# mkshing/e4t-diffusion

Measured on NVIDIA H100. Metric: E4T pretrain images/sec @512^2 bs16 SD-v1.4, higher is better.
Workload: dtype bf16

## Files before the change

e4t-diffusion_b200/csrc/common.cuh:

```cuda
#pragma once
#include <cuda.h>
#include <cuda_runtime.h>
#include <cuda_bf16.h>
#include <stdint.h>
#include <stdio.h>
#include <string.h>

typedef __nv_bfloat16 bf16;

extern thread_local char g_e4t_err[512];
int e4t_set_error(const char* fmt, ...);

#define E4T_CHECK(cond, ...)                                   \
  do {                                                         \
    if (!(cond)) return e4t_set_error(__VA_ARGS__);            \
  } while (0)

#define E4T_CUDA(call)                                                                  \
  do {                                                                                  \
    cudaError_t _e = (call);                                                            \
    if (_e != cudaSuccess)                                                              \
      return e4t_set_error("%s:%d CUDA error %s: %s", __FILE__, __LINE__, #call,        \
                           cudaGetErrorString(_e));                                     \
  } while (0)

#define E4T_LAUNCH_CHECK() E4T_CUDA(cudaGetLastError())

extern unsigned long long g_e4t_launches;
#define E4T_COUNT_LAUNCH() (++g_e4t_launches)

int e4t_tmap_encode(CUtensorMap* map, const void* gptr, int rank, const uint64_t* dims,
                    const uint64_t* strides_bytes ,
                    const uint32_t* box, int elem_bytes , int swizzle_bytes = 128,
                    const uint32_t* elem_strides = nullptr );

static inline int cdiv(long a, long b) { return (int)((a + b - 1) / b); }

#ifdef __CUDACC__
__device__ __forceinline__ uint32_t smem_u32(const void* p) {
  return static_cast<uint32_t>(__cvta_generic_to_shared(p));
}
__device__ __forceinline__ uint32_t lane_id() { return threadIdx.x & 31; }

__device__ __forceinline__ void mbar_init(uint64_t* bar, uint32_t count) {
  asm volatile("mbarrier.init.shared::cta.b64 [%0], %1;" ::"r"(smem_u32(bar)), "r"(count) : "memory");
}
__device__ __forceinline__ void fence_mbar_init() {
  asm volatile("fence.mbarrier_init.release.cluster;" ::: "memory");
}
__device__ __forceinline__ void mbar_expect_tx(uint64_t* bar, uint32_t bytes) {
  asm volatile("mbarrier.arrive.expect_tx.shared::cta.b64 _, [%0], %1;" ::"r"(smem_u32(bar)), "r"(bytes)
               : "memory");
}
__device__ __forceinline__ void mbar_arrive(uint64_t* bar) {
  asm volatile("mbarrier.arrive.shared::cta.b64 _, [%0];" ::"r"(smem_u32(bar)) : "memory");
}
__device__ __forceinline__ bool mbar_try_wait(uint64_t* bar, uint32_t parity) {
  uint32_t ok;
  asm volatile(
      "{\n\t.reg .pred p;\n\t"
      "mbarrier.try_wait.parity.shared::cta.b64 p, [%1], %2;\n\t"
      "selp.u32 %0, 1, 0, p;\n\t}"
      : "=r"(ok)
      : "r"(smem_u32(bar)), "r"(parity)
      : "memory");
  return ok != 0;
}
__device__ __forceinline__ bool mbar_test_wait(uint64_t* bar, uint32_t parity) {
  uint32_t ok;
  asm volatile(
      "{\n\t.reg .pred p;\n\t"
      "mbarrier.test_wait.parity.shared::cta.b64 p, [%1], %2;\n\t"
      "selp.u32 %0, 1, 0, p;\n\t}"
      : "=r"(ok)
      : "r"(smem_u32(bar)), "r"(parity)
      : "memory");
  return ok != 0;
}
__device__ __forceinline__ void mbar_wait(uint64_t* bar, uint32_t parity) {
  while (!mbar_try_wait(bar, parity)) {
  }
}

__device__ __forceinline__ void fence_proxy_async_smem() {
  asm volatile("fence.proxy.async.shared::cta;" ::: "memory");
}

__device__ __forceinline__ void tma_prefetch_desc(const CUtensorMap* m) {
  asm volatile("prefetch.tensormap [%0];" ::"l"(reinterpret_cast<uint64_t>(m)) : "memory");
}
__device__ __forceinline__ void tma_load_2d(void* smem, const CUtensorMap* m, uint64_t* bar, int c0, int c1) {
  asm volatile(
      "cp.async.bulk.tensor.2d.shared::cluster.global.mbarrier::complete_tx::bytes [%0], [%1, {%3, %4}], [%2];"
      ::"r"(smem_u32(smem)), "l"(reinterpret_cast<uint64_t>(m)), "r"(smem_u32(bar)), "r"(c0), "r"(c1)
      : "memory");
}
__device__ __forceinline__ void tma_load_3d(void* smem, const CUtensorMap* m, uint64_t* bar, int c0, int c1,
                                            int c2) {
  asm volatile(
      "cp.async.bulk.tensor.3d.shared::cluster.global.mbarrier::complete_tx::bytes [%0], [%1, {%3, %4, %5}], [%2];"
      ::"r"(smem_u32(smem)), "l"(reinterpret_cast<uint64_t>(m)), "r"(smem_u32(bar)), "r"(c0), "r"(c1), "r"(c2)
      : "memory");
}
__device__ __forceinline__ void tma_load_4d(void* smem, const CUtensorMap* m, uint64_t* bar, int c0, int c1,
                                            int c2, int c3) {
  asm volatile(
      "cp.async.bulk.tensor.4d.shared::cluster.global.mbarrier::complete_tx::bytes [%0], [%1, {%3, %4, %5, %6}], "
      "[%2];" ::"r"(smem_u32(smem)),
      "l"(reinterpret_cast<uint64_t>(m)), "r"(smem_u32(bar)), "r"(c0), "r"(c1), "r"(c2), "r"(c3)
      : "memory");
}

__device__ __forceinline__ void bulk_load_1d(void* smem, const void* g, uint32_t bytes, uint64_t* bar) {
  asm volatile("cp.async.bulk.shared::cluster.global.mbarrier::complete_tx::bytes [%0], [%1], %2, [%3];" ::"r"(
                   smem_u32(smem)),
               "l"(g), "r"(bytes), "r"(smem_u32(bar))
               : "memory");
}

__device__ __forceinline__ void tma_store_3d(const CUtensorMap* m, const void* smem, int c0, int c1, int c2) {
  asm volatile("cp.async.bulk.tensor.3d.global.shared::cta.bulk_group [%0, {%2, %3, %4}], [%1];" ::"l"(
                   reinterpret_cast<uint64_t>(m)),
               "r"(smem_u32(smem)), "r"(c0), "r"(c1), "r"(c2)
               : "memory");
}
__device__ __forceinline__ void tma_reduce_add_3d(const CUtensorMap* m, const void* smem, int c0, int c1, int c2) {
  asm volatile("cp.reduce.async.bulk.tensor.3d.global.shared::cta.add.tile.bulk_group [%0, {%2, %3, %4}], [%1];" ::"l"(
                   reinterpret_cast<uint64_t>(m)),
               "r"(smem_u32(smem)), "r"(c0), "r"(c1), "r"(c2)
               : "memory");
}
__device__ __forceinline__ void tma_store_commit() { asm volatile("cp.async.bulk.commit_group;" ::: "memory"); }
template <int N>
__device__ __forceinline__ void tma_store_wait_read() {
  asm volatile("cp.async.bulk.wait_group.read %0;" ::"n"(N) : "memory");
}
__device__ __forceinline__ void tma_store_wait_all() { asm volatile("cp.async.bulk.wait_group 0;" ::: "memory"); }

__device__ __forceinline__ uint64_t wgmma_desc(uint32_t saddr, uint32_t lbo_bytes, uint32_t sbo_bytes) {
  uint64_t d = 0;
  d |= (uint64_t)((saddr & 0x3FFFFu) >> 4);
  d |= (uint64_t)((lbo_bytes >> 4) & 0x3FFFu) << 16;
  d |= (uint64_t)((sbo_bytes >> 4) & 0x3FFFu) << 32;
  d |= 1ull << 62;
  return d;
}
__device__ __forceinline__ void wgmma_fence() { asm volatile("wgmma.fence.sync.aligned;" ::: "memory"); }
__device__ __forceinline__ void wgmma_commit() { asm volatile("wgmma.commit_group.sync.aligned;" ::: "memory"); }
template <int N>
__device__ __forceinline__ void wgmma_wait() {
  asm volatile("wgmma.wait_group.sync.aligned %0;" ::"n"(N) : "memory");
}
template <int R>
__device__ __forceinline__ void reg_fence(float* d) {
#pragma unroll
  for (int i = 0; i < R; ++i) asm volatile("" : "+f"(d[i])::"memory");
}
template <int R>
__device__ __forceinline__ void reg_fence_u32(uint32_t* a) {
#pragma unroll
  for (int i = 0; i < R; ++i) asm volatile("" : "+r"(a[i])::"memory");
}
__device__ __forceinline__ void named_bar_sync(uint32_t id, uint32_t nthreads) {
  asm volatile("bar.sync %0, %1;" ::"r"(id), "r"(nthreads) : "memory");
}
template <int R>
__device__ __forceinline__ void setmaxnreg_dec() {
  asm volatile("setmaxnreg.dec.sync.aligned.u32 %0;" ::"n"(R));
}
template <int R>
__device__ __forceinline__ void setmaxnreg_inc() {
  asm volatile("setmaxnreg.inc.sync.aligned.u32 %0;" ::"n"(R));
}

__device__ __forceinline__ void ldsm_x4(uint32_t addr, uint32_t* r) {
  asm volatile("ldmatrix.sync.aligned.m8n8.x4.shared.b16 {%0, %1, %2, %3}, [%4];"
               : "=r"(r[0]), "=r"(r[1]), "=r"(r[2]), "=r"(r[3])
               : "r"(addr));
}
__device__ __forceinline__ void ldsm_x4_t(uint32_t addr, uint32_t* r) {
  asm volatile("ldmatrix.sync.aligned.m8n8.x4.trans.shared.b16 {%0, %1, %2, %3}, [%4];"
               : "=r"(r[0]), "=r"(r[1]), "=r"(r[2]), "=r"(r[3])
               : "r"(addr));
}
__device__ __forceinline__ void mma16816(float* d, const uint32_t* a, const uint32_t* b) {
  asm volatile(
      "mma.sync.aligned.m16n8k16.row.col.f32.bf16.bf16.f32 {%0, %1, %2, %3}, {%4, %5, %6, %7}, {%8, %9}, "
      "{%0, %1, %2, %3};"
      : "+f"(d[0]), "+f"(d[1]), "+f"(d[2]), "+f"(d[3])
      : "r"(a[0]), "r"(a[1]), "r"(a[2]), "r"(a[3]), "r"(b[0]), "r"(b[1]));
}
__device__ __forceinline__ void cp_async16(uint32_t dst, const void* src, uint32_t src_bytes) {
  asm volatile("cp.async.cg.shared.global [%0], [%1], 16, %2;" ::"r"(dst), "l"(src), "r"(src_bytes) : "memory");
}
__device__ __forceinline__ void cp_async_commit() { asm volatile("cp.async.commit_group;" ::: "memory"); }
template <int N>
__device__ __forceinline__ void cp_async_wait() {
  asm volatile("cp.async.wait_group %0;" ::"n"(N) : "memory");
}

__device__ __forceinline__ uint32_t sw128_off(uint32_t r, uint32_t c16) {
  return r * 128u + ((c16 ^ (r & 7u)) << 4);
}

__device__ __forceinline__ float warp_sum(float v) {
#pragma unroll
  for (int o = 16; o > 0; o >>= 1) v += __shfl_xor_sync(0xffffffffu, v, o);
  return v;
}
__device__ __forceinline__ float warp_max(float v) {
#pragma unroll
  for (int o = 16; o > 0; o >>= 1) v = fmaxf(v, __shfl_xor_sync(0xffffffffu, v, o));
  return v;
}
__device__ __forceinline__ uint32_t pack_bf16(float a, float b) {
  __nv_bfloat162 t = __floats2bfloat162_rn(a, b);
  return *reinterpret_cast<uint32_t*>(&t);
}
__device__ __forceinline__ float2 unpack_bf16(uint32_t u) {
  __nv_bfloat162 t = *reinterpret_cast<__nv_bfloat162*>(&u);
  return __bfloat1622float2(t);
}
__device__ __forceinline__ float ex2_approx(float x) {
  float y;
  asm("ex2.approx.ftz.f32 %0, %1;" : "=f"(y) : "f"(x));
  return y;
}
__device__ __forceinline__ float silu_f(float x) { return x / (1.f + __expf(-x)); }
#endif
```

e4t-diffusion_b200/csrc/gemm.cu:

```cuda
#include "common.cuh"
#include "wgmma.cuh"
#include <stdlib.h>

struct GemmArgs {
  int M, N, K, batch;
  int BN, m_tiles, n_tiles, splits, kchunks, kper, stages;
  int a_mn, b_mn, a_batched, b_batched;
  int conv, H, W, BH, BB, cin_chunks, cout;
  int cstride;
  int cpad;
  void* out;
  int out_mode;
  long long ldo, out_bstride;
  const float* bias;
  const float* rowgroup;
  int rows_per_group;
  const bf16* residual;
  long long ldr, res_bstride;
  float alpha;
  int pair_store;
  int epi_tma;
};

static constexpr int kBM = 128;
static constexpr int kBK = 64;
static constexpr int kATileBytes = kBM * kBK * 2;
static constexpr int kThreads = 384;
static constexpr int kSubBytes = 64 * 64;
template <int BN>
constexpr int kStgBytes = 64 * BN * 2;

__device__ __forceinline__ void gemm_decode(const GemmArgs& g, long t, int& n_t, int& m_t, int& sp, int& bz) {
  n_t = (int)(t % g.n_tiles);
  long r = t / g.n_tiles;
  m_t = (int)(r % g.m_tiles);
  r /= g.m_tiles;
  sp = (int)(r % g.splits);
  bz = (int)(r / g.splits);
}

template <int BN, int AMN, int BMN>
__device__ __forceinline__ void gemm_epilogue(const GemmArgs& g, const float* acc, int m_t, int n0, int bz, int wg_row) {
  const int lane = threadIdx.x & 31;
  const int w = (threadIdx.x >> 5) & 3;
#pragma unroll
  for (int h = 0; h < 2; ++h) {
    const int m = m_t * kBM + wg_row + w * 16 + (lane >> 2) + 8 * h;
    if (m >= g.M) continue;
    const float* rg = g.rowgroup ? g.rowgroup + (long long)(m / g.rows_per_group) * g.N : nullptr;
    const bf16* res = g.residual ? g.residual + (long long)bz * g.res_bstride + (long long)m * g.ldr : nullptr;
    const long long orow = (long long)bz * g.out_bstride + (long long)m * g.ldo;
#pragma unroll
    for (int j = 0; j < BN / 8; ++j) {
      const int n = n0 + 8 * j + 2 * (lane & 3);
      if (n >= g.N) break;
      float f0 = acc[4 * j + 2 * h] * g.alpha, f1 = acc[4 * j + 2 * h + 1] * g.alpha;
      const bool two = n + 1 < g.N;
      if (g.bias) { f0 += g.bias[n]; if (two) f1 += g.bias[n + 1]; }
      if (rg) { f0 += rg[n]; if (two) f1 += rg[n + 1]; }
      if (res) { f0 += __bfloat162float(res[n]); if (two) f1 += __bfloat162float(res[n + 1]); }
      if (g.out_mode == 0) {
        bf16* o = reinterpret_cast<bf16*>(g.out) + orow + n;
        if (two && g.pair_store) {
          *reinterpret_cast<uint32_t*>(o) = pack_bf16(f0, f1);
        } else {
          o[0] = __float2bfloat16(f0);
          if (two) o[1] = __float2bfloat16(f1);
        }
      } else if (g.out_mode == 1) {
        float* o = reinterpret_cast<float*>(g.out) + orow + n;
        if (two && g.pair_store) {
          *reinterpret_cast<float2*>(o) = make_float2(f0, f1);
        } else {
          o[0] = f0;
          if (two) o[1] = f1;
        }
      } else {
        float* o = reinterpret_cast<float*>(g.out) + orow + n;
        atomicAdd(o, f0);
        if (two) atomicAdd(o + 1, f1);
      }
    }
  }
}

template <int BN, typename OutT>
__device__ __forceinline__ void gemm_epilogue_tma(const GemmArgs& g, const CUtensorMap* mapO, const float* acc,
                                                  uint8_t* stg, int m_t, int n0, int bz, int wg_row, uint32_t bar_id) {
  constexpr int kEsz = (int)sizeof(OutT);
  constexpr int kSubCols = 64 / kEsz;
  constexpr int kSubsPerPass = kStgBytes<BN> / kSubBytes;
  constexpr int kPasses = BN / kSubCols / kSubsPerPass;
  const int tid = threadIdx.x & 127;
  const int lane = tid & 31;
  const int w = tid >> 5;
  const int row0 = m_t * kBM + wg_row;
#pragma unroll
  for (int p = 0; p < kPasses; ++p) {
    if (tid == 0) tma_store_wait_read<0>();
    named_bar_sync(bar_id, 128);
#pragma unroll
    for (int h = 0; h < 2; ++h) {
      const int r = w * 16 + (lane >> 2) + 8 * h;
      const int m = row0 + r;
      if (m >= g.M) continue;
      const float* rg = g.rowgroup ? g.rowgroup + (long long)(m / g.rows_per_group) * g.N : nullptr;
      const bf16* res = g.residual ? g.residual + (long long)bz * g.res_bstride + (long long)m * g.ldr : nullptr;
      uint8_t* srow = stg + r * 64;
      const int sw = (r >> 1) & 3;
#pragma unroll
      for (int j = 0; j < BN / 8; ++j) {
        const int sub = 8 * j / kSubCols;
        if (sub / kSubsPerPass != p) continue;
        const int n = n0 + 8 * j + 2 * (lane & 3);
        float f0 = acc[4 * j + 2 * h] * g.alpha, f1 = acc[4 * j + 2 * h + 1] * g.alpha;
        if (n < g.N) {
          const bool two = n + 1 < g.N;
          if (g.bias) { f0 += g.bias[n]; if (two) f1 += g.bias[n + 1]; }
          if (rg) { f0 += rg[n]; if (two) f1 += rg[n + 1]; }
          if (res) { f0 += __bfloat162float(res[n]); if (two) f1 += __bfloat162float(res[n + 1]); }
        }
        const int byte = (8 * j % kSubCols + 2 * (lane & 3)) * kEsz;
        uint8_t* dst = srow + (sub % kSubsPerPass) * kSubBytes + ((((byte >> 4) ^ sw)) << 4) + (byte & 15);
        if (kEsz == 2) *reinterpret_cast<uint32_t*>(dst) = pack_bf16(f0, f1);
        else *reinterpret_cast<float2*>(dst) = make_float2(f0, f1);
      }
    }
    fence_proxy_async_smem();
    named_bar_sync(bar_id, 128);
    if (tid == 0 && row0 < g.M) {
#pragma unroll 1
      for (int s = 0; s < kSubsPerPass; ++s) {
        const int n = n0 + (p * kSubsPerPass + s) * kSubCols;
        if (n >= g.N) break;
        if (g.out_mode == 2) tma_reduce_add_3d(mapO, stg + s * kSubBytes, n, row0, bz);
        else tma_store_3d(mapO, stg + s * kSubBytes, n, row0, bz);
      }
      tma_store_commit();
    }
  }
}

template <int BN, int AMN, int BMN>
__global__ void __launch_bounds__(kThreads, 1)
e4t_gemm_kernel(const __grid_constant__ CUtensorMap mapA, const __grid_constant__ CUtensorMap mapB,
                const __grid_constant__ CUtensorMap mapO, const GemmArgs g) {
  extern __shared__ __align__(1024) uint8_t smem_raw[];
  uint8_t* smem = smem_raw + ((1024u - (smem_u32(smem_raw) & 1023u)) & 1023u);
  constexpr int kBTileBytes = BN * kBK * 2;
  constexpr int kStageBytes = kATileBytes + kBTileBytes;
  uint8_t* staging = smem + (size_t)g.stages * kStageBytes;
  uint64_t* full_bar = reinterpret_cast<uint64_t*>(staging + 2 * kStgBytes<BN>);
  uint64_t* empty_bar = full_bar + g.stages;

  const int wg = threadIdx.x >> 7;
  if (threadIdx.x == 0) {
    tma_prefetch_desc(&mapA);
    tma_prefetch_desc(&mapB);
    if (g.epi_tma) tma_prefetch_desc(&mapO);
    for (int i = 0; i < g.stages; ++i) {
      mbar_init(&full_bar[i], 1);
      mbar_init(&empty_bar[i], 256);
    }
    fence_mbar_init();
  }
  __syncthreads();

  const long total_tiles = (long)g.batch * g.splits * g.m_tiles * g.n_tiles;

  if (wg == 0) {
    setmaxnreg_dec<40>();
    if (threadIdx.x != 0) return;
    int s = 0;
    uint32_t ph = 0;
    for (long t = blockIdx.x; t < total_tiles; t += gridDim.x) {
      int n_t, m_t, sp, bz;
      gemm_decode(g, t, n_t, m_t, sp, bz);
      const int m0 = m_t * kBM, n0 = n_t * BN;
      const int kc0 = sp * g.kper;
      const int kc1 = min(g.kchunks, kc0 + g.kper);
      int cb0 = 0, ch0 = 0, cw0 = 0;
      if (g.conv == 1) {
        const int img = g.H * g.W;
        cb0 = m0 / img;
        ch0 = (m0 % img) / g.W;
        cw0 = m0 % g.W;
      }
      for (int kc = kc0; kc < kc1; ++kc) {
        mbar_wait(&empty_bar[s], ph ^ 1u);
        uint8_t* sA = smem + (size_t)s * kStageBytes;
        uint8_t* sB = sA + kATileBytes;
        mbar_expect_tx(&full_bar[s], (uint32_t)kStageBytes);
        if (g.conv == 2) {
          const int tap = bz, dy = tap / 3, dx = tap % 3;
          const int p0 = kc * kBK, img = g.H * g.W;
          const int b0 = p0 / img, h0 = (p0 % img) / g.W;
          tma_load_3d(sA, &mapA, &full_bar[s], m0, p0, 0);
          tma_load_3d(sA + 8192, &mapA, &full_bar[s], m0 + 64, p0, 0);
          for (int i = 0; i < BN / 64; ++i)
            tma_load_4d(sB + i * 8192, &mapB, &full_bar[s], n0 + 64 * i, dx - 1, h0 + dy - 1, b0);
        } else if (g.conv) {
          const int tap = kc / g.cin_chunks, cc = kc % g.cin_chunks;
          const int dy = tap / 3, dx = tap % 3;
          tma_load_4d(sA, &mapA, &full_bar[s], cc * kBK, g.cstride * cw0 + dx - g.cpad, g.cstride * ch0 + dy - g.cpad,
                      cb0);
          tma_load_2d(sB, &mapB, &full_bar[s], cc * kBK, tap * g.cout + n0);
        } else {
          const int ab = g.a_batched ? bz : 0, bb = g.b_batched ? bz : 0;
          if (!AMN) {
            tma_load_3d(sA, &mapA, &full_bar[s], kc * kBK, m0, ab);
          } else {
            tma_load_3d(sA, &mapA, &full_bar[s], m0, kc * kBK, ab);
            tma_load_3d(sA + 8192, &mapA, &full_bar[s], m0 + 64, kc * kBK, ab);
          }
          if (!BMN) {
            tma_load_3d(sB, &mapB, &full_bar[s], kc * kBK, n0, bb);
          } else {
            for (int i = 0; i < BN / 64; ++i)
              tma_load_3d(sB + i * 8192, &mapB, &full_bar[s], n0 + 64 * i, kc * kBK, bb);
          }
        }
        if (++s == g.stages) {
          s = 0;
          ph ^= 1u;
        }
      }
    }
  } else {
    setmaxnreg_inc<232>();
    const int wg_row = (wg - 1) * 64;
    const uint32_t s0 = smem_u32(smem);
    const uint64_t dA0 = AMN ? wgmma_desc(s0 + 8192u * (wg - 1), 8192, 1024)
                             : wgmma_desc(s0 + 8192u * (wg - 1), 16, 1024);
    const uint64_t dB0 = BMN ? wgmma_desc(s0 + kATileBytes, 8192, 1024) : wgmma_desc(s0 + kATileBytes, 16, 1024);
    constexpr uint32_t a_step = AMN ? (2048u >> 4) : (32u >> 4);
    constexpr uint32_t b_step = BMN ? (2048u >> 4) : (32u >> 4);
    constexpr uint32_t stage_units = (uint32_t)kStageBytes >> 4;
    float acc[BN / 2];
    int s = 0;
    uint32_t ph = 0;
    for (long t = blockIdx.x; t < total_tiles; t += gridDim.x) {
      int n_t, m_t, sp, bz;
      gemm_decode(g, t, n_t, m_t, sp, bz);
      const int kc0 = sp * g.kper;
      const int kc1 = min(g.kchunks, kc0 + g.kper);
      int prev = -1;
      for (int kc = kc0; kc < kc1; ++kc) {
        mbar_wait(&full_bar[s], ph);
        const uint64_t da = dA0 + (uint64_t)((uint32_t)s * stage_units);
        const uint64_t db = dB0 + (uint64_t)((uint32_t)s * stage_units);
        reg_fence<BN / 2>(acc);
        wgmma_fence();
#pragma unroll
        for (int k = 0; k < kBK / 16; ++k)
          Wgmma<BN, AMN, BMN>::mma(acc, da + (uint64_t)(k * a_step), db + (uint64_t)(k * b_step),
                                   (kc > kc0 || k > 0) ? 1u : 0u);
        wgmma_commit();
        reg_fence<BN / 2>(acc);
        wgmma_wait<1>();
        reg_fence<BN / 2>(acc);
        if (prev >= 0) mbar_arrive(&empty_bar[prev]);
        prev = s;
        if (++s == g.stages) {
          s = 0;
          ph ^= 1u;
        }
      }
      wgmma_wait<0>();
      reg_fence<BN / 2>(acc);
      if (prev >= 0) mbar_arrive(&empty_bar[prev]);
      if (!g.epi_tma) {
        gemm_epilogue<BN, AMN, BMN>(g, acc, m_t, n_t * BN, bz, wg_row);
      } else {
        uint8_t* stg = staging + (wg - 1) * kStgBytes<BN>;
        if (g.out_mode == 0) gemm_epilogue_tma<BN, bf16>(g, &mapO, acc, stg, m_t, n_t * BN, bz, wg_row, wg);
        else gemm_epilogue_tma<BN, float>(g, &mapO, acc, stg, m_t, n_t * BN, bz, wg_row, wg);
      }
    }
    if (g.epi_tma && (threadIdx.x & 127) == 0) tma_store_wait_all();
  }
}

static int g_num_sms = 0;
static int num_sms() {
  if (g_num_sms == 0) {
    int dev = 0;
    cudaGetDevice(&dev);
    cudaDeviceGetAttribute(&g_num_sms, cudaDevAttrMultiProcessorCount, dev);
    if (g_num_sms <= 0) g_num_sms = 132;
  }
  return g_num_sms;
}

static int pick_bn(int N, long m_tiles_x_batch, bool b_mn, int force_bn, int kchunks_per_tile = 16,
                   bool residual = false, bool atomic = false, double* cost_out = nullptr) {
  if (force_bn > 0) return force_bn;
  const int step = b_mn ? 64 : 32;
  int best = 0;
  double best_cost = 1e30;
  const double sms = (double)num_sms();
  for (int bn = 256; bn >= 64; bn -= step) {
    const int tiles_n = cdiv(N, bn);
    const double tiles = (double)tiles_n * (double)m_tiles_x_batch;
    const double mainloop = kchunks_per_tile * (160.0 + 3.9 * bn);
    const double epilogue = 600.0 + 12.0 * bn * (residual ? 2.0 : 1.0) * (atomic ? 4.0 : 1.0);
    const double rounds = (double)((long)((tiles + sms - 1) / sms));
    const double cost = rounds * (mainloop + epilogue);
    if (cost < best_cost - 1e-6) {
      best_cost = cost;
      best = bn;
    }
  }
  if (cost_out) *cost_out = best_cost;
  return best;
}

static int auto_splits(int N, long m_tiles_x_batch, bool b_mn, int kchunks) {
  int best = 1;
  double best_cost = 1e30;
  const int smax = kchunks < 64 ? kchunks : 64;
  for (int sp = 1; sp <= smax; ++sp) {
    const int kper = cdiv(kchunks, sp);
    if (cdiv(kchunks, kper) != sp) continue;
    double c = 0;
    pick_bn(N, m_tiles_x_batch * sp, b_mn, 0, kper, false, true, &c);
    if (c < best_cost - 1e-6) {
      best_cost = c;
      best = sp;
    }
  }
  return best;
}

template <int BN, int AMN, int BMN>
static int launch_gemm_t(const CUtensorMap& mA, const CUtensorMap& mB, const CUtensorMap& mO, GemmArgs& g, int grid,
                         cudaStream_t stream) {
  constexpr int stage_bytes = kATileBytes + BN * kBK * 2;
  int stages = (227 * 1024 - 1024 - 2 * kStgBytes<BN> - 16 * (int)sizeof(uint64_t)) / stage_bytes;
  if (stages > 8) stages = 8;
  if (stages > g.kper) stages = g.kper < 2 ? 2 : g.kper;
  g.stages = stages;
  const size_t smem = (size_t)stages * stage_bytes + 2 * kStgBytes<BN> + 2 * stages * sizeof(uint64_t) + 1024;
  static bool attr_set = false;
  if (!attr_set) {
    E4T_CUDA(cudaFuncSetAttribute(e4t_gemm_kernel<BN, AMN, BMN>, cudaFuncAttributeMaxDynamicSharedMemorySize,
                                  227 * 1024));
    attr_set = true;
  }
  e4t_gemm_kernel<BN, AMN, BMN><<<grid, kThreads, smem, stream>>>(mA, mB, mO, g);
  E4T_COUNT_LAUNCH();
  E4T_LAUNCH_CHECK();
  return 0;
}

template <int AMN, int BMN>
static int launch_gemm_bn(const CUtensorMap& mA, const CUtensorMap& mB, const CUtensorMap& mO, GemmArgs& g, int grid,
                          cudaStream_t stream) {
  switch (g.BN) {
    case 64: return launch_gemm_t<64, AMN, BMN>(mA, mB, mO, g, grid, stream);
    case 128: return launch_gemm_t<128, AMN, BMN>(mA, mB, mO, g, grid, stream);
    case 192: return launch_gemm_t<192, AMN, BMN>(mA, mB, mO, g, grid, stream);
    case 256: return launch_gemm_t<256, AMN, BMN>(mA, mB, mO, g, grid, stream);
  }
  if (!BMN) {
    switch (g.BN) {
      case 96: return launch_gemm_t<96, AMN, 0>(mA, mB, mO, g, grid, stream);
      case 160: return launch_gemm_t<160, AMN, 0>(mA, mB, mO, g, grid, stream);
      case 224: return launch_gemm_t<224, AMN, 0>(mA, mB, mO, g, grid, stream);
    }
  }
  return e4t_set_error("e4t_gemm_bf16: unsupported tile width BN=%d (b_mn=%d)", g.BN, BMN);
}

static int launch_gemm(const CUtensorMap& mA, const CUtensorMap& mB, GemmArgs& g, cudaStream_t stream) {
  const int esz = g.out_mode == 0 ? 2 : 4;
  g.pair_store = (g.ldo % 2) == 0 && (g.batch == 1 || (g.out_bstride % 2) == 0) && ((uintptr_t)g.out % (2 * esz)) == 0;
  const char* p = getenv("E4T_GEMM_EPI_PLAIN");
  const bool want_tma = !(p && *p) || atoi(p) != 0;
  g.epi_tma = want_tma && ((uintptr_t)g.out % 16) == 0 && (g.ldo * esz) % 16 == 0 && g.ldo >= g.N &&
              (g.batch == 1 || (g.out_bstride > 0 && (g.out_bstride * esz) % 16 == 0));
  CUtensorMap mO;
  memset(&mO, 0, sizeof(mO));
  if (g.epi_tma) {
    const uint64_t bs = g.batch == 1 ? (uint64_t)g.ldo * g.M : (uint64_t)g.out_bstride;
    uint64_t dims[3] = {(uint64_t)g.N, (uint64_t)g.M, (uint64_t)g.batch};
    uint64_t str[2] = {(uint64_t)g.ldo * esz, bs * esz};
    uint32_t box[3] = {(uint32_t)(64 / esz), 64, 1};
    if (int e = e4t_tmap_encode(&mO, g.out, 3, dims, str, box, esz, 64)) return e;
  }
  const long total = (long)g.batch * g.splits * g.m_tiles * g.n_tiles;
  int grid = (int)(total < num_sms() ? total : num_sms());
  if (grid < 1) return 0;
  if (g.a_mn)
    return g.b_mn ? launch_gemm_bn<1, 1>(mA, mB, mO, g, grid, stream) : launch_gemm_bn<1, 0>(mA, mB, mO, g, grid, stream);
  return g.b_mn ? launch_gemm_bn<0, 1>(mA, mB, mO, g, grid, stream) : launch_gemm_bn<0, 0>(mA, mB, mO, g, grid, stream);
}

extern "C" int e4t_gemm_bf16(const void* A, const void* B, void* out, int M, int N, int K, int batch, int a_mn,
                             int b_mn, long long lda, long long ldb, long long a_bstride, long long b_bstride,
                             int out_mode, long long ldo, long long out_bstride, const float* bias,
                             const float* rowgroup, int rows_per_group, const void* residual, long long ldr,
                             long long res_bstride, float alpha, int splits, int force_bn, void* stream_) {
  cudaStream_t stream = (cudaStream_t)stream_;
  E4T_CHECK(M > 0 && N > 0 && K > 0 && batch > 0, "e4t_gemm_bf16: bad dims M=%d N=%d K=%d batch=%d", M, N, K, batch);
  E4T_CHECK((lda % 8) == 0 && (ldb % 8) == 0, "e4t_gemm_bf16: leading strides must be multiples of 8 elements");
  E4T_CHECK(((uintptr_t)A % 16) == 0 && ((uintptr_t)B % 16) == 0, "e4t_gemm_bf16: operands must be 16-byte aligned");
  E4T_CHECK(out_mode >= 0 && out_mode <= 2, "e4t_gemm_bf16: bad out_mode");
  GemmArgs g;
  memset(&g, 0, sizeof(g));
  g.M = M; g.N = N; g.K = K; g.batch = batch;
  g.a_mn = a_mn; g.b_mn = b_mn;
  g.a_batched = (a_bstride != 0); g.b_batched = (b_bstride != 0);
  g.m_tiles = cdiv(M, kBM);
  g.kchunks = cdiv(K, kBK);
  if (splits == 0 && out_mode == 2 && force_bn <= 0) splits = auto_splits(N, (long)g.m_tiles * batch, b_mn != 0, g.kchunks);
  if (splits < 1) splits = 1;
  if (splits > g.kchunks) splits = g.kchunks;
  g.kper = cdiv(g.kchunks, splits);
  g.splits = cdiv(g.kchunks, g.kper);
  g.BN = pick_bn(N, (long)g.m_tiles * batch * g.splits, b_mn != 0, force_bn, g.kper, residual != nullptr, out_mode == 2);
  E4T_CHECK(g.BN >= 64 && g.BN <= 256 && (g.BN % (b_mn ? 64 : 32)) == 0, "e4t_gemm_bf16: bad BN %d", g.BN);
  g.n_tiles = cdiv(N, g.BN);
  E4T_CHECK(g.splits == 1 || out_mode == 2, "e4t_gemm_bf16: split-K requires atomic fp32 output");
  g.out = out; g.out_mode = out_mode; g.ldo = ldo; g.out_bstride = out_bstride;
  g.bias = bias; g.rowgroup = rowgroup; g.rows_per_group = rows_per_group > 0 ? rows_per_group : 1;
  g.residual = (const bf16*)residual; g.ldr = ldr; g.res_bstride = res_bstride;
  g.alpha = alpha;

  CUtensorMap mA, mB;
  {
    const uint64_t nb = g.a_batched ? (uint64_t)batch : 1;
    const uint64_t bs = g.a_batched ? (uint64_t)a_bstride : (uint64_t)lda * (a_mn ? K : M);
    if (!a_mn) {
      uint64_t dims[3] = {(uint64_t)K, (uint64_t)M, nb};
      uint64_t str[2] = {(uint64_t)lda * 2, bs * 2};
      uint32_t box[3] = {kBK, kBM, 1};
      if (int e = e4t_tmap_encode(&mA, A, 3, dims, str, box, 2)) return e;
    } else {
      uint64_t dims[3] = {(uint64_t)M, (uint64_t)K, nb};
      uint64_t str[2] = {(uint64_t)lda * 2, bs * 2};
      uint32_t box[3] = {64, kBK, 1};
      if (int e = e4t_tmap_encode(&mA, A, 3, dims, str, box, 2)) return e;
    }
  }
  {
    const uint64_t nb = g.b_batched ? (uint64_t)batch : 1;
    const uint64_t bs = g.b_batched ? (uint64_t)b_bstride : (uint64_t)ldb * (b_mn ? K : N);
    if (!b_mn) {
      uint64_t dims[3] = {(uint64_t)K, (uint64_t)N, nb};
      uint64_t str[2] = {(uint64_t)ldb * 2, bs * 2};
      uint32_t box[3] = {kBK, (uint32_t)g.BN, 1};
      if (int e = e4t_tmap_encode(&mB, B, 3, dims, str, box, 2)) return e;
    } else {
      uint64_t dims[3] = {(uint64_t)N, (uint64_t)K, nb};
      uint64_t str[2] = {(uint64_t)ldb * 2, bs * 2};
      uint32_t box[3] = {64, kBK, 1};
      if (int e = e4t_tmap_encode(&mB, B, 3, dims, str, box, 2)) return e;
    }
  }
  return launch_gemm(mA, mB, g, stream);
}

static int conv3x3_impl(const void* x, const void* w, void* out, int B, int Hin, int Win, int Cin, int Cout, int stride,
                        int pad_lo, int out_mode, const float* bias, const float* rowgroup, const void* residual,
                        int force_bn, cudaStream_t stream) {
  E4T_CHECK(Cin % 64 == 0, "e4t_conv3x3: Cin must be a multiple of 64 (got %d)", Cin);
  E4T_CHECK(stride == 1 || (stride == 2 && Hin % 2 == 0 && Win % 2 == 0), "e4t_conv3x3: bad stride/size");
  E4T_CHECK(pad_lo == 1 || (stride == 2 && pad_lo == 0), "e4t_conv3x3: bad padding %d for stride %d", pad_lo, stride);
  const int H = Hin / stride, W = Win / stride;
  const bool wide = W > 128;
  E4T_CHECK((W <= 128 && (128 % W) == 0) || (wide && W % 128 == 0),
            "e4t_conv3x3: output width must divide 128 or be a multiple of 128 (got %d)", W);
  E4T_CHECK(out_mode == 0 || out_mode == 1, "e4t_conv3x3: bad out_mode");
  const int img = H * W;
  int BH, BB;
  if (wide) {
    BB = 1;
    BH = 1;
  } else if (img >= 128) {
    BB = 1;
    BH = 128 / W;
    E4T_CHECK(H % BH == 0, "e4t_conv3x3: H=%d not a multiple of tile height %d", H, BH);
  } else {
    E4T_CHECK(128 % img == 0, "e4t_conv3x3: H*W must divide 128");
    BB = 128 / img;
    BH = H;
  }
  const int BW = wide ? 128 : W;
  GemmArgs g;
  memset(&g, 0, sizeof(g));
  g.M = B * img; g.N = Cout; g.K = Cin; g.batch = 1;
  g.conv = 1; g.H = H; g.W = W; g.BH = BH; g.BB = BB; g.cin_chunks = Cin / 64; g.cout = Cout; g.cstride = stride;
  g.cpad = pad_lo;
  g.m_tiles = cdiv(g.M, kBM);
  g.kchunks = 9 * g.cin_chunks;
  g.kper = g.kchunks; g.splits = 1;
  g.BN = pick_bn(Cout, g.m_tiles, false, force_bn, g.kchunks, residual != nullptr, false);
  g.n_tiles = cdiv(Cout, g.BN);
  g.out = out; g.out_mode = out_mode; g.ldo = Cout; g.out_bstride = 0;
  g.bias = bias; g.rowgroup = rowgroup; g.rows_per_group = img;
  g.residual = (const bf16*)residual; g.ldr = Cout; g.res_bstride = 0;
  g.alpha = 1.f;
  CUtensorMap mA, mB;
  {
    uint64_t dims[4] = {(uint64_t)Cin, (uint64_t)Win, (uint64_t)Hin, (uint64_t)B};
    uint64_t str[3] = {(uint64_t)Cin * 2, (uint64_t)Win * Cin * 2, (uint64_t)Hin * Win * Cin * 2};
    uint32_t box[4] = {kBK, (uint32_t)(BW * stride), (uint32_t)(BH * stride), (uint32_t)BB};
    uint32_t es[4] = {1, (uint32_t)stride, (uint32_t)stride, 1};
    if (int e = e4t_tmap_encode(&mA, x, 4, dims, str, box, 2, 128, stride == 1 ? nullptr : es)) return e;
  }
  {
    uint64_t dims[2] = {(uint64_t)Cin, (uint64_t)9 * Cout};
    uint64_t str[1] = {(uint64_t)Cin * 2};
    uint32_t box[2] = {kBK, (uint32_t)g.BN};
    if (int e = e4t_tmap_encode(&mB, w, 2, dims, str, box, 2)) return e;
  }
  return launch_gemm(mA, mB, g, stream);
}

extern "C" int e4t_conv3x3_bf16(const void* x, const void* w, void* out, int B, int H, int W, int Cin, int Cout,
                                int out_mode, const float* bias, const float* rowgroup, const void* residual,
                                int force_bn, void* stream_) {
  return conv3x3_impl(x, w, out, B, H, W, Cin, Cout, 1, 1, out_mode, bias, rowgroup, residual, force_bn,
                      (cudaStream_t)stream_);
}

extern "C" int e4t_conv3x3_s2_bf16(const void* x, const void* w, void* out, int B, int H, int W, int Cin, int Cout,
                                   const float* bias, int force_bn, void* stream_) {
  return conv3x3_impl(x, w, out, B, H, W, Cin, Cout, 2, 1, 0, bias, nullptr, nullptr, force_bn, (cudaStream_t)stream_);
}

extern "C" int e4t_conv3x3_s2p_bf16(const void* x, const void* w, void* out, int B, int H, int W, int Cin, int Cout,
                                    int pad_lo, const float* bias, int force_bn, void* stream_) {
  return conv3x3_impl(x, w, out, B, H, W, Cin, Cout, 2, pad_lo, 0, bias, nullptr, nullptr, force_bn,
                      (cudaStream_t)stream_);
}

extern "C" int e4t_conv3x3_wgrad(const void* x, const void* dy, float* dw9, int B, int H, int W, int Cin, int Cout,
                                 void* stream_) {
  cudaStream_t stream = (cudaStream_t)stream_;
  E4T_CHECK(Cin % 64 == 0 && Cout % 64 == 0, "e4t_conv3x3_wgrad: Cin, Cout must be multiples of 64 (%d, %d)", Cin, Cout);
  E4T_CHECK(W <= 64 && (64 % W) == 0 && (H * W) % 64 == 0 && H % (64 / W) == 0,
            "e4t_conv3x3_wgrad: unsupported image %dx%d (W | 64, H*W %% 64 == 0)", H, W);
  const long long pixels = (long long)B * H * W;
  GemmArgs g;
  memset(&g, 0, sizeof(g));
  g.M = Cout; g.N = Cin; g.K = (int)pixels; g.batch = 9;
  g.a_mn = 1; g.b_mn = 1; g.a_batched = 0; g.b_batched = 1;
  g.conv = 2; g.H = H; g.W = W; g.cout = Cout; g.cstride = 1; g.cpad = 1;
  g.m_tiles = cdiv(Cout, kBM);
  g.kchunks = (int)(pixels / kBK);
  const int base_tiles = 9 * g.m_tiles * cdiv(Cin, 256);
  int splits = cdiv(2 * num_sms(), base_tiles);
  if (splits < 1) splits = 1;
  if (splits > g.kchunks) splits = g.kchunks;
  g.kper = cdiv(g.kchunks, splits);
  g.splits = cdiv(g.kchunks, g.kper);
  g.BN = Cin >= 256 ? 256 : (Cin >= 192 ? 192 : (Cin >= 128 ? 128 : 64));
  g.n_tiles = cdiv(Cin, g.BN);
  g.out = dw9; g.out_mode = 2; g.ldo = Cin; g.out_bstride = (long long)Cout * Cin;
  g.rows_per_group = 1; g.alpha = 1.f;
  CUtensorMap mA, mB;
  {
    uint64_t dims[3] = {(uint64_t)Cout, (uint64_t)pixels, 1};
    uint64_t str[2] = {(uint64_t)Cout * 2, (uint64_t)pixels * Cout * 2};
    uint32_t box[3] = {64, kBK, 1};
    if (int e = e4t_tmap_encode(&mA, dy, 3, dims, str, box, 2)) return e;
  }
  {
    uint64_t dims[4] = {(uint64_t)Cin, (uint64_t)W, (uint64_t)H, (uint64_t)B};
    uint64_t str[3] = {(uint64_t)Cin * 2, (uint64_t)W * Cin * 2, (uint64_t)H * W * Cin * 2};
    uint32_t box[4] = {64, (uint32_t)W, (uint32_t)(64 / W), 1};
    if (int e = e4t_tmap_encode(&mB, x, 4, dims, str, box, 2)) return e;
  }
  return launch_gemm(mA, mB, g, stream);
}
```

Before: 100.1.

## Add ping-pong consumer warpgroup schedule to the wgmma GEMM and conv kernels

Adds a ping-pong mode in which each consumer warpgroup computes a full 128-row tile and the two warpgroups alternate tiles. Named barriers order their mainloops so one warpgroup's epilogue overlaps the other's MMA. The BN picker gets a cost model that chooses ping-pong for long-K tiles with BN of 160 or less, preferring it when there is an epilogue addend. This doubles the accumulator registers per warpgroup and adds new phase-tracking and barrier logic across skipped tiles, which risks register pressure and synchronization bugs.

```diff
diff --git a/e4t-diffusion_b200/csrc/common.cuh b/e4t-diffusion_b200/csrc/common.cuh
--- a/e4t-diffusion_b200/csrc/common.cuh
+++ b/e4t-diffusion_b200/csrc/common.cuh
@@ -164,6 +164,9 @@
 __device__ __forceinline__ void named_bar_sync(uint32_t id, uint32_t nthreads) {
   asm volatile("bar.sync %0, %1;" ::"r"(id), "r"(nthreads) : "memory");
 }
+__device__ __forceinline__ void named_bar_arrive(uint32_t id, uint32_t nthreads) {
+  asm volatile("bar.arrive %0, %1;" ::"r"(id), "r"(nthreads) : "memory");
+}
 template <int R>
 __device__ __forceinline__ void setmaxnreg_dec() {
   asm volatile("setmaxnreg.dec.sync.aligned.u32 %0;" ::"n"(R));
diff --git a/e4t-diffusion_b200/csrc/gemm.cu b/e4t-diffusion_b200/csrc/gemm.cu
--- a/e4t-diffusion_b200/csrc/gemm.cu
+++ b/e4t-diffusion_b200/csrc/gemm.cu
@@ -20,12 +20,16 @@
   float alpha;
   int pair_store;
   int epi_tma;
+  int pingpong;
 };
 
 static constexpr int kBM = 128;
 static constexpr int kBK = 64;
 static constexpr int kATileBytes = kBM * kBK * 2;
 static constexpr int kThreads = 384;
+static constexpr int kOrderBar = 3;
+template <int PP>
+constexpr int kWgRows = PP ? 128 : 64;
 static constexpr int kSubBytes = 64 * 64;
 template <int BN>
 constexpr int kStgBytes = 64 * BN * 2;
@@ -84,7 +88,7 @@
   }
 }
 
-template <int BN, typename OutT>
+template <int BN, int PP, typename OutT>
 __device__ __forceinline__ void gemm_epilogue_tma(const GemmArgs& g, const CUtensorMap* mapO, const float* acc,
                                                   uint8_t* stg, int m_t, int n0, int bz, int wg_row, uint32_t bar_id) {
   constexpr int kEsz = (int)sizeof(OutT);
@@ -94,54 +98,58 @@
   const int tid = threadIdx.x & 127;
   const int lane = tid & 31;
   const int w = tid >> 5;
-  const int row0 = m_t * kBM + wg_row;
-#pragma unroll
-  for (int p = 0; p < kPasses; ++p) {
-    if (tid == 0) tma_store_wait_read<0>();
-    named_bar_sync(bar_id, 128);
-#pragma unroll
-    for (int h = 0; h < 2; ++h) {
-      const int r = w * 16 + (lane >> 2) + 8 * h;
-      const int m = row0 + r;
-      if (m >= g.M) continue;
-      const float* rg = g.rowgroup ? g.rowgroup + (long long)(m / g.rows_per_group) * g.N : nullptr;
-      const bf16* res = g.residual ? g.residual + (long long)bz * g.res_bstride + (long long)m * g.ldr : nullptr;
-      uint8_t* srow = stg + r * 64;
-      const int sw = (r >> 1) & 3;
-#pragma unroll
-      for (int j = 0; j < BN / 8; ++j) {
-        const int sub = 8 * j / kSubCols;
-        if (sub / kSubsPerPass != p) continue;
-        const int n = n0 + 8 * j + 2 * (lane & 3);
-        float f0 = acc[4 * j + 2 * h] * g.alpha, f1 = acc[4 * j + 2 * h + 1] * g.alpha;
-        if (n < g.N) {
-          const bool two = n + 1 < g.N;
-          if (g.bias) { f0 += g.bias[n]; if (two) f1 += g.bias[n + 1]; }
-          if (rg) { f0 += rg[n]; if (two) f1 += rg[n + 1]; }
-          if (res) { f0 += __bfloat162float(res[n]); if (two) f1 += __bfloat162float(res[n + 1]); }
-        }
-        const int byte = (8 * j % kSubCols + 2 * (lane & 3)) * kEsz;
-        uint8_t* dst = srow + (sub % kSubsPerPass) * kSubBytes + ((((byte >> 4) ^ sw)) << 4) + (byte & 15);
-        if (kEsz == 2) *reinterpret_cast<uint32_t*>(dst) = pack_bf16(f0, f1);
-        else *reinterpret_cast<float2*>(dst) = make_float2(f0, f1);
-      }
-    }
-    fence_proxy_async_smem();
-    named_bar_sync(bar_id, 128);
-    if (tid == 0 && row0 < g.M) {
+#pragma unroll
+  for (int mb = 0; mb < kWgRows<PP> / 64; ++mb) {
+    const int row0 = m_t * kBM + wg_row + mb * 64;
+    const float* a = acc + mb * (BN / 2);
+#pragma unroll
+    for (int p = 0; p < kPasses; ++p) {
+      if (tid == 0) tma_store_wait_read<0>();
+      named_bar_sync(bar_id, 128);
+#pragma unroll
+      for (int h = 0; h < 2; ++h) {
+        const int r = w * 16 + (lane >> 2) + 8 * h;
+        const int m = row0 + r;
+        if (m >= g.M) continue;
+        const float* rg = g.rowgroup ? g.rowgroup + (long long)(m / g.rows_per_group) * g.N : nullptr;
+        const bf16* res = g.residual ? g.residual + (long long)bz * g.res_bstride + (long long)m * g.ldr : nullptr;
+        uint8_t* srow = stg + r * 64;
+        const int sw = (r >> 1) & 3;
+#pragma unroll
+        for (int j = 0; j < BN / 8; ++j) {
+          const int sub = 8 * j / kSubCols;
+          if (sub / kSubsPerPass != p) continue;
+          const int n = n0 + 8 * j + 2 * (lane & 3);
+          float f0 = a[4 * j + 2 * h] * g.alpha, f1 = a[4 * j + 2 * h + 1] * g.alpha;
+          if (n < g.N) {
+            const bool two = n + 1 < g.N;
+            if (g.bias) { f0 += g.bias[n]; if (two) f1 += g.bias[n + 1]; }
+            if (rg) { f0 += rg[n]; if (two) f1 += rg[n + 1]; }
+            if (res) { f0 += __bfloat162float(res[n]); if (two) f1 += __bfloat162float(res[n + 1]); }
+          }
+          const int byte = (8 * j % kSubCols + 2 * (lane & 3)) * kEsz;
+          uint8_t* dst = srow + (sub % kSubsPerPass) * kSubBytes + ((((byte >> 4) ^ sw)) << 4) + (byte & 15);
+          if (kEsz == 2) *reinterpret_cast<uint32_t*>(dst) = pack_bf16(f0, f1);
+          else *reinterpret_cast<float2*>(dst) = make_float2(f0, f1);
+        }
+      }
+      fence_proxy_async_smem();
+      named_bar_sync(bar_id, 128);
+      if (tid == 0 && row0 < g.M) {
 #pragma unroll 1
-      for (int s = 0; s < kSubsPerPass; ++s) {
-        const int n = n0 + (p * kSubsPerPass + s) * kSubCols;
-        if (n >= g.N) break;
-        if (g.out_mode == 2) tma_reduce_add_3d(mapO, stg + s * kSubBytes, n, row0, bz);
-        else tma_store_3d(mapO, stg + s * kSubBytes, n, row0, bz);
-      }
-      tma_store_commit();
-    }
-  }
-}
-
-template <int BN, int AMN, int BMN>
+        for (int s = 0; s < kSubsPerPass; ++s) {
+          const int n = n0 + (p * kSubsPerPass + s) * kSubCols;
+          if (n >= g.N) break;
+          if (g.out_mode == 2) tma_reduce_add_3d(mapO, stg + s * kSubBytes, n, row0, bz);
+          else tma_store_3d(mapO, stg + s * kSubBytes, n, row0, bz);
+        }
+        tma_store_commit();
+      }
+    }
+  }
+}
+
+template <int BN, int AMN, int BMN, int PP>
 __global__ void __launch_bounds__(kThreads, 1)
 e4t_gemm_kernel(const __grid_constant__ CUtensorMap mapA, const __grid_constant__ CUtensorMap mapB,
                 const __grid_constant__ CUtensorMap mapO, const GemmArgs g) {
@@ -160,7 +168,7 @@
     if (g.epi_tma) tma_prefetch_desc(&mapO);
     for (int i = 0; i < g.stages; ++i) {
       mbar_init(&full_bar[i], 1);
-      mbar_init(&empty_bar[i], 256);
+      mbar_init(&empty_bar[i], PP ? 128 : 256);
     }
     fence_mbar_init();
   }
@@ -228,37 +236,53 @@
     }
   } else {
     setmaxnreg_inc<232>();
-    const int wg_row = (wg - 1) * 64;
+    const int me = wg - 1;
+    const int wg_row = PP ? 0 : me * 64;
+    constexpr int kMB = kWgRows<PP> / 64;
+    constexpr int kAcc = kMB * BN / 2;
     const uint32_t s0 = smem_u32(smem);
-    const uint64_t dA0 = AMN ? wgmma_desc(s0 + 8192u * (wg - 1), 8192, 1024)
-                             : wgmma_desc(s0 + 8192u * (wg - 1), 16, 1024);
+    const uint32_t a0 = s0 + 8192u * (uint32_t)(wg_row / 64);
+    const uint64_t dA0 = AMN ? wgmma_desc(a0, 8192, 1024) : wgmma_desc(a0, 16, 1024);
     const uint64_t dB0 = BMN ? wgmma_desc(s0 + kATileBytes, 8192, 1024) : wgmma_desc(s0 + kATileBytes, 16, 1024);
     constexpr uint32_t a_step = AMN ? (2048u >> 4) : (32u >> 4);
     constexpr uint32_t b_step = BMN ? (2048u >> 4) : (32u >> 4);
     constexpr uint32_t stage_units = (uint32_t)kStageBytes >> 4;
-    float acc[BN / 2];
+    constexpr uint32_t mb_units = 8192u >> 4;
+    float acc[kAcc];
     int s = 0;
     uint32_t ph = 0;
-    for (long t = blockIdx.x; t < total_tiles; t += gridDim.x) {
+    int local = 0;
+    for (long t = blockIdx.x; t < total_tiles; t += gridDim.x, ++local) {
       int n_t, m_t, sp, bz;
       gemm_decode(g, t, n_t, m_t, sp, bz);
       const int kc0 = sp * g.kper;
       const int kc1 = min(g.kchunks, kc0 + g.kper);
+      if (PP) {
+        if ((local & 1) != me) {
+          const int ns = s + (kc1 - kc0);
+          ph ^= (uint32_t)((ns / g.stages) & 1);
+          s = ns % g.stages;
+          continue;
+        }
+        if (local > 0) named_bar_sync(kOrderBar + me, 256);
+      }
       int prev = -1;
       for (int kc = kc0; kc < kc1; ++kc) {
         mbar_wait(&full_bar[s], ph);
         const uint64_t da = dA0 + (uint64_t)((uint32_t)s * stage_units);
         const uint64_t db = dB0 + (uint64_t)((uint32_t)s * stage_units);
-        reg_fence<BN / 2>(acc);
+        reg_fence<kAcc>(acc);
         wgmma_fence();
 #pragma unroll
         for (int k = 0; k < kBK / 16; ++k)
-          Wgmma<BN, AMN, BMN>::mma(acc, da + (uint64_t)(k * a_step), db + (uint64_t)(k * b_step),
-                                   (kc > kc0 || k > 0) ? 1u : 0u);
+#pragma unroll
+          for (int mb = 0; mb < kMB; ++mb)
+            Wgmma<BN, AMN, BMN>::mma(acc + mb * (BN / 2), da + (uint64_t)(k * a_step + mb * mb_units),
+                                     db + (uint64_t)(k * b_step), (kc > kc0 || k > 0) ? 1u : 0u);
         wgmma_commit();
-        reg_fence<BN / 2>(acc);
+        reg_fence<kAcc>(acc);
         wgmma_wait<1>();
-        reg_fence<BN / 2>(acc);
+        reg_fence<kAcc>(acc);
         if (prev >= 0) mbar_arrive(&empty_bar[prev]);
         prev = s;
         if (++s == g.stages) {
@@ -266,15 +290,18 @@
           ph ^= 1u;
         }
       }
+      if (PP && t + gridDim.x < total_tiles) named_bar_arrive(kOrderBar + (me ^ 1), 256);
       wgmma_wait<0>();
-      reg_fence<BN / 2>(acc);
+      reg_fence<kAcc>(acc);
       if (prev >= 0) mbar_arrive(&empty_bar[prev]);
       if (!g.epi_tma) {
-        gemm_epilogue<BN, AMN, BMN>(g, acc, m_t, n_t * BN, bz, wg_row);
+#pragma unroll
+        for (int mb = 0; mb < kMB; ++mb)
+          gemm_epilogue<BN, AMN, BMN>(g, acc + mb * (BN / 2), m_t, n_t * BN, bz, wg_row + mb * 64);
       } else {
-        uint8_t* stg = staging + (wg - 1) * kStgBytes<BN>;
-        if (g.out_mode == 0) gemm_epilogue_tma<BN, bf16>(g, &mapO, acc, stg, m_t, n_t * BN, bz, wg_row, wg);
-        else gemm_epilogue_tma<BN, float>(g, &mapO, acc, stg, m_t, n_t * BN, bz, wg_row, wg);
+        uint8_t* stg = staging + me * kStgBytes<BN>;
+        if (g.out_mode == 0) gemm_epilogue_tma<BN, PP, bf16>(g, &mapO, acc, stg, m_t, n_t * BN, bz, wg_row, wg);
+        else gemm_epilogue_tma<BN, PP, float>(g, &mapO, acc, stg, m_t, n_t * BN, bz, wg_row, wg);
       }
     }
     if (g.epi_tma && (threadIdx.x & 127) == 0) tma_store_wait_all();
@@ -292,26 +319,40 @@
   return g_num_sms;
 }
 
+static constexpr int kPingPongMinChunks = 10;
+static constexpr int kPingPongPlainChunks = 40;
 static int pick_bn(int N, long m_tiles_x_batch, bool b_mn, int force_bn, int kchunks_per_tile = 16,
-                   bool residual = false, bool atomic = false, double* cost_out = nullptr) {
-  if (force_bn > 0) return force_bn;
+                   bool residual = false, bool atomic = false, double* cost_out = nullptr, int* pingpong = nullptr,
+                   bool addend = false) {
+  const bool pp_ok = kchunks_per_tile > kPingPongMinChunks && (addend || kchunks_per_tile >= kPingPongPlainChunks);
   const int step = b_mn ? 64 : 32;
-  int best = 0;
+  int best = 0, best_pp = 0;
   double best_cost = 1e30;
   const double sms = (double)num_sms();
   for (int bn = 256; bn >= 64; bn -= step) {
+    if (force_bn > 0 && bn != force_bn) continue;
     const int tiles_n = cdiv(N, bn);
     const double tiles = (double)tiles_n * (double)m_tiles_x_batch;
     const double mainloop = kchunks_per_tile * (160.0 + 3.9 * bn);
-    const double epilogue = 600.0 + 12.0 * bn * (residual ? 2.0 : 1.0) * (atomic ? 4.0 : 1.0);
+    const double epi_scale = (residual ? 2.0 : 1.0) * (atomic ? 4.0 : 1.0);
+    const double epilogue = 600.0 + 12.0 * bn * epi_scale;
     const double rounds = (double)((long)((tiles + sms - 1) / sms));
-    const double cost = rounds * (mainloop + epilogue);
-    if (cost < best_cost - 1e-6) {
-      best_cost = cost;
-      best = bn;
-    }
-  }
+    for (int pp = 0; pp <= (bn <= 160 && pp_ok ? 1 : 0); ++pp) {
+      double cost = rounds * (mainloop + epilogue);
+      if (pp) {
+        const double epi_pp = 600.0 + 24.0 * bn * epi_scale;
+        cost = rounds * mainloop + epi_pp + (rounds - 1.0) * 0.5 * fmax(0.0, epi_pp - mainloop);
+      }
+      if (cost < best_cost - 1e-6) {
+        best_cost = cost;
+        best = bn;
+        best_pp = pp;
+      }
+    }
+  }
+  if (force_bn > 0 && best == 0) best = force_bn;
   if (cost_out) *cost_out = best_cost;
+  if (pingpong) *pingpong = best_pp;
   return best;
 }
 
@@ -332,22 +373,23 @@
   return best;
 }
 
-template <int BN, int AMN, int BMN>
+template <int BN, int AMN, int BMN, int PP>
 static int launch_gemm_t(const CUtensorMap& mA, const CUtensorMap& mB, const CUtensorMap& mO, GemmArgs& g, int grid,
                          cudaStream_t stream) {
   constexpr int stage_bytes = kATileBytes + BN * kBK * 2;
-  int stages = (227 * 1024 - 1024 - 2 * kStgBytes<BN> - 16 * (int)sizeof(uint64_t)) / stage_bytes;
+  constexpr int stg_bytes = 2 * kStgBytes<BN>;
+  int stages = (227 * 1024 - 1024 - stg_bytes - 16 * (int)sizeof(uint64_t)) / stage_bytes;
   if (stages > 8) stages = 8;
   if (stages > g.kper) stages = g.kper < 2 ? 2 : g.kper;
   g.stages = stages;
-  const size_t smem = (size_t)stages * stage_bytes + 2 * kStgBytes<BN> + 2 * stages * sizeof(uint64_t) + 1024;
+  const size_t smem = (size_t)stages * stage_bytes + stg_bytes + 2 * stages * sizeof(uint64_t) + 1024;
   static bool attr_set = false;
   if (!attr_set) {
-    E4T_CUDA(cudaFuncSetAttribute(e4t_gemm_kernel<BN, AMN, BMN>, cudaFuncAttributeMaxDynamicSharedMemorySize,
+    E4T_CUDA(cudaFuncSetAttribute(e4t_gemm_kernel<BN, AMN, BMN, PP>, cudaFuncAttributeMaxDynamicSharedMemorySize,
                                   227 * 1024));
     attr_set = true;
   }
-  e4t_gemm_kernel<BN, AMN, BMN><<<grid, kThreads, smem, stream>>>(mA, mB, mO, g);
+  e4t_gemm_kernel<BN, AMN, BMN, PP><<<grid, kThreads, smem, stream>>>(mA, mB, mO, g);
   E4T_COUNT_LAUNCH();
   E4T_LAUNCH_CHECK();
   return 0;
@@ -356,17 +398,30 @@
 template <int AMN, int BMN>
 static int launch_gemm_bn(const CUtensorMap& mA, const CUtensorMap& mB, const CUtensorMap& mO, GemmArgs& g, int grid,
                           cudaStream_t stream) {
+  if (g.pingpong) {
+    switch (g.BN) {
+      case 64: return launch_gemm_t<64, AMN, BMN, 1>(mA, mB, mO, g, grid, stream);
+      case 128: return launch_gemm_t<128, AMN, BMN, 1>(mA, mB, mO, g, grid, stream);
+    }
+    if (!BMN) {
+      switch (g.BN) {
+        case 96: return launch_gemm_t<96, AMN, 0, 1>(mA, mB, mO, g, grid, stream);
+        case 160: return launch_gemm_t<160, AMN, 0, 1>(mA, mB, mO, g, grid, stream);
+      }
+    }
+    return e4t_set_error("e4t_gemm_bf16: unsupported ping-pong tile width BN=%d (b_mn=%d)", g.BN, BMN);
+  }
   switch (g.BN) {
-    case 64: return launch_gemm_t<64, AMN, BMN>(mA, mB, mO, g, grid, stream);
-    case 128: return launch_gemm_t<128, AMN, BMN>(mA, mB, mO, g, grid, stream);
-    case 192: return launch_gemm_t<192, AMN, BMN>(mA, mB, mO, g, grid, stream);
-    case 256: return launch_gemm_t<256, AMN, BMN>(mA, mB, mO, g, grid, stream);
+    case 64: return launch_gemm_t<64, AMN, BMN, 0>(mA, mB, mO, g, grid, stream);
+    case 128: return launch_gemm_t<128, AMN, BMN, 0>(mA, mB, mO, g, grid, stream);
+    case 192: return launch_gemm_t<192, AMN, BMN, 0>(mA, mB, mO, g, grid, stream);
+    case 256: return launch_gemm_t<256, AMN, BMN, 0>(mA, mB, mO, g, grid, stream);
   }
   if (!BMN) {
     switch (g.BN) {
-      case 96: return launch_gemm_t<96, AMN, 0>(mA, mB, mO, g, grid, stream);
-      case 160: return launch_gemm_t<160, AMN, 0>(mA, mB, mO, g, grid, stream);
-      case 224: return launch_gemm_t<224, AMN, 0>(mA, mB, mO, g, grid, stream);
+      case 96: return launch_gemm_t<96, AMN, 0, 0>(mA, mB, mO, g, grid, stream);
+      case 160: return launch_gemm_t<160, AMN, 0, 0>(mA, mB, mO, g, grid, stream);
+      case 224: return launch_gemm_t<224, AMN, 0, 0>(mA, mB, mO, g, grid, stream);
     }
   }
   return e4t_set_error("e4t_gemm_bf16: unsupported tile width BN=%d (b_mn=%d)", g.BN, BMN);
@@ -418,7 +473,8 @@
   if (splits > g.kchunks) splits = g.kchunks;
   g.kper = cdiv(g.kchunks, splits);
   g.splits = cdiv(g.kchunks, g.kper);
-  g.BN = pick_bn(N, (long)g.m_tiles * batch * g.splits, b_mn != 0, force_bn, g.kper, residual != nullptr, out_mode == 2);
+  g.BN = pick_bn(N, (long)g.m_tiles * batch * g.splits, b_mn != 0, force_bn, g.kper, residual != nullptr, out_mode == 2,
+                 nullptr, &g.pingpong, bias || rowgroup || residual);
   E4T_CHECK(g.BN >= 64 && g.BN <= 256 && (g.BN % (b_mn ? 64 : 32)) == 0, "e4t_gemm_bf16: bad BN %d", g.BN);
   g.n_tiles = cdiv(N, g.BN);
   E4T_CHECK(g.splits == 1 || out_mode == 2, "e4t_gemm_bf16: split-K requires atomic fp32 output");
@@ -495,7 +551,8 @@
   g.m_tiles = cdiv(g.M, kBM);
   g.kchunks = 9 * g.cin_chunks;
   g.kper = g.kchunks; g.splits = 1;
-  g.BN = pick_bn(Cout, g.m_tiles, false, force_bn, g.kchunks, residual != nullptr, false);
+  g.BN = pick_bn(Cout, g.m_tiles, false, force_bn, g.kchunks, residual != nullptr, false, nullptr, &g.pingpong,
+                 bias || rowgroup || residual);
   g.n_tiles = cdiv(Cout, g.BN);
   g.out = out; g.out_mode = out_mode; g.ldo = Cout; g.out_bstride = 0;
   g.bias = bias; g.rowgroup = rowgroup; g.rows_per_group = img;
```

After: 102.0, median of 6. +1.9%, better.
